# morisUtokyo/mTR

Measured on AMD Instinct MI355X. Metric: reads/sec, 2 kb Nanopore synthetic, higher is better.
Workload: dtype int32

## Files before the change

### mtr_amd/__init__.py

```python
from __future__ import annotations

import ctypes as C
import os
from typing import List, NamedTuple, Sequence

import numpy as np

HERE = os.path.dirname(os.path.abspath(__file__))
LIB_PATH = os.environ.get("MTR_LIB", os.path.join(HERE, "libmtr_hip.so"))
MAX_PERIOD = 500
MAX_READ_LENGTH = 833333
TEXT_ASCII, TEXT_CODES = 0, 1
FASTA_TILE_BYTES = 4096
FASTA_END = {0: "eof", 1: "empty", 2: "bad", 3: "toolong"}
FASTQ_END = {**FASTA_END, 4: "format", 5: "more"}

STATUS = {0: "MTR_OK", 1: "MTR_ERR_NO_DEVICE", 2: "MTR_ERR_BAD_ARG", 3: "MTR_ERR_OOM", 4: "MTR_ERR_HIP",
          5: "MTR_ERR_OVERFLOW", 6: "MTR_ERR_DP_TOO_LARGE"}
COUNTER_NAMES = ["dp_calls", "dp_cells", "dp_rows", "revise_dp_calls", "revise_dp_cells", "kmer_tables", "kmer_lookups",
                 "ranges_candidate", "ranges_executed", "records", "di_passes", "di_positions", "traceback_steps",
                 "undefined_guards", "global_tables", "reserved",
                 "cyc_total", "cyc_dp_fwd", "cyc_dp_tb", "cyc_tab_build", "cyc_seeds", "cyc_walk", "cyc_polish", "cyc_revise_vote",
                 "cyc_slot_copy", "cyc_dp_fwd_rev", "cyc_dp_tb_rev", "cyc_k1_codes", "cyc_k1_passes", "cyc_k1_extract",
                 "cyc_k1_dedup", "cyc_k1_total",
                 "memo_hits", "memo_cells", "tables_skipped", "cyc_tb_refill", "tb_refills", "walk_steps", "walk_slow_steps", "cyc_walk_slow",
                 "walk_calls", "walk_closed", "cyc_walk_fast", "prof43", "prof44", "prof45", "prof46", "prof47",
                 "qpass_bytes_dp2", "qpass_cells_dp2", "qpass_bytes_rev", "qpass_cells_rev", "revisions_shared", "reads_sent_back", "ranges_searched", "prof55"]
EXPORTS = ["mtr_create", "mtr_destroy", "mtr_last_error", "mtr_abi_version", "mtr_process_batch", "mtr_free_results",
           "mtr_upload_batch", "mtr_run_resident", "mtr_fetch_results", "mtr_get_kernel_times", "mtr_get_counters",
           "mtr_test_ranges", "mtr_test_ranges_parts", "mtr_test_wrap_dp", "mtr_test_wrap_dp_pass", "mtr_test_polish", "mtr_test_revise", "mtr_test_last_mode", "mtr_set_trace", "mtr_get_trace",
           "mtr_run_resident_async", "mtr_wait", "mtr_alignments",
           "mtr_file_state_create", "mtr_file_state_destroy", "mtr_upload_batch_in_file", "mtr_file_state_skip",
           "mtr_get_bases_after_read", "mtr_upload_batch_packed", "mtr_fetch_results_packed", "mtr_export_packed_device",
           "mtr_unpack_records", "mtr_pack_records", "mtr_get_first_failed_read", "mtr_upload_batch_device",
           "mtr_report_device", "mtr_test_chain", "mtr_report_alignments_device", "mtr_report_text_device", "mtr_test_report_lines",
           "mtr_parse_fasta_device", "mtr_upload_fasta_device", "mtr_fasta_index",
           "mtr_parse_fastq_device", "mtr_upload_fastq_device", "mtr_upload_fastq_device_in_file",
           "mtr_upload_batch_device_in_file", "mtr_upload_fasta_device_in_file", "mtr_file_state_skip_device", "mtr_test_file_tail",
           "mtr_parse_fasta_device_window", "mtr_upload_fasta_device_window", "mtr_parse_fastq_device_window", "mtr_upload_fastq_device_window",
           "mtr_report_motifs_device", "mtr_test_unit_motifs", "mtr_search_motifs_device",
           "mtr_search_motif_loci_device", "mtr_motif_loci_copy_device", "mtr_search_flanks_device", "mtr_genotype_loci_device",
           "mtr_call_alleles_device", "mtr_genotype_partial_device", "mtr_genotype_catalog_device", "mtr_genotype_catalog_copy_device",
           "mtr_call_alleles_rows_device", "mtr_test_catalog_stats", "mtr_genotype_partial_catalog_device", "mtr_genotype_partial_catalog_copy_device",
           "mtr_test_partial_catalog_stats", "mtr_catalog_create", "mtr_catalog_destroy", "mtr_catalog_info_get", "mtr_genotype_catalog_prepared_device",
           "mtr_genotype_partial_catalog_prepared_device", "mtr_test_catalog_dump", "mtr_test_catalog_build_stats",
           "mtr_extract_windows_device", "mtr_allele_consensus_device", "mtr_window_structure_device",
           "mtr_window_edits_device", "mtr_window_edits_copy_device", "mtr_test_window_edits_rounds"]
WE_FIELDS = 6
WS_MAX_SEGMENTS, WS_MAX_WINDOW = 4, 16384
CONS_MAX_WINDOW, CONS_MAX_BAND, CONS_INS_SLOTS, CONS_MAX_EXTRA = 16384, 256, 4, 64
ALLELE_COPIES, ALLELE_BASES = 0, 1
ALIGN_WIDTH = 50


class MtrError(RuntimeError):
    pass


class FileState:

    def __init__(self):
        self.lib = load_library()
        h = C.c_void_p()
        st = self.lib.mtr_file_state_create(C.byref(h))
        if st != 0:
            raise MtrError(f"mtr_file_state_create: {STATUS.get(st, st)}")
        self.h = h

    def skip(self, reads):
        bases, offs, lens = _flatten(reads)
        st = self.lib.mtr_file_state_skip(self.h, bases.ctypes.data, offs.ctypes.data, lens.ctypes.data, len(reads))
        if st != 0:
            raise MtrError(f"mtr_file_state_skip: {STATUS.get(st, st)}")

    def skip_device(self, engine: "Engine", text, offsets, lens, codes: bool = False):
        import torch

        offs, ln = device_input_args(text, offsets, lens, engine.device)
        stream = torch.cuda.current_stream(text.device).cuda_stream
        engine._check(self.lib.mtr_file_state_skip_device(engine.h, self.h, C.c_void_p(text.data_ptr()), text.numel(), offs.ctypes.data, ln.ctypes.data,
                                                          len(ln), TEXT_CODES if codes else TEXT_ASCII, C.c_void_p(stream)), "mtr_file_state_skip_device")

    def close(self):
# ... 401 lines not shown
    if not os.path.exists(path):
        raise MtrError(f"{path} is missing: build it with `python -m mtr_amd.build` (hipcc, gfx950); there is no CPU fallback")
    lib = C.CDLL(path)
    P = C.POINTER
    lib.mtr_create.argtypes = [C.c_int, C.c_int, C.c_float, P(C.c_void_p)]
    lib.mtr_create.restype = C.c_int
    lib.mtr_destroy.argtypes = [C.c_void_p]
    lib.mtr_destroy.restype = None
    lib.mtr_last_error.argtypes = [C.c_void_p]
    lib.mtr_last_error.restype = C.c_char_p
    lib.mtr_abi_version.restype = C.c_int
    lib.mtr_process_batch.argtypes = [C.c_void_p, C.c_void_p, C.c_void_p, C.c_void_p, C.c_int32, P(P(CRecord)), P(P(C.c_int32)), P(C.c_int64)]
    lib.mtr_process_batch.restype = C.c_int
    lib.mtr_free_results.argtypes = [C.c_void_p, C.c_void_p]
    lib.mtr_free_results.restype = None
    lib.mtr_upload_batch.argtypes = [C.c_void_p, C.c_void_p, C.c_void_p, C.c_void_p, C.c_int32]
    lib.mtr_upload_batch.restype = C.c_int
    lib.mtr_run_resident.argtypes = [C.c_void_p]
    lib.mtr_run_resident.restype = C.c_int
    lib.mtr_file_state_create.argtypes = [P(C.c_void_p)]
    lib.mtr_file_state_create.restype = C.c_int
    lib.mtr_file_state_destroy.argtypes = [C.c_void_p]
    lib.mtr_file_state_destroy.restype = None
    lib.mtr_upload_batch_in_file.argtypes = [C.c_void_p, C.c_void_p, C.c_void_p, C.c_void_p, C.c_void_p, C.c_int32]
    lib.mtr_upload_batch_in_file.restype = C.c_int
    lib.mtr_file_state_skip.argtypes = [C.c_void_p, C.c_void_p, C.c_void_p, C.c_void_p, C.c_int32]
    lib.mtr_file_state_skip.restype = C.c_int
    lib.mtr_run_resident_async.argtypes = [C.c_void_p]
    lib.mtr_run_resident_async.restype = C.c_int
    lib.mtr_wait.argtypes = [C.c_void_p]
    lib.mtr_wait.restype = C.c_int
    lib.mtr_test_last_mode.argtypes = [C.c_void_p]
    lib.mtr_test_last_mode.restype = C.c_int32
    lib.mtr_fetch_results.argtypes = [C.c_void_p, P(P(CRecord)), P(P(C.c_int32)), P(C.c_int64)]
    lib.mtr_fetch_results.restype = C.c_int
    lib.mtr_get_kernel_times.argtypes = [C.c_void_p, P(CKernelTime), C.c_int32]
    lib.mtr_get_kernel_times.restype = C.c_int
    lib.mtr_alignments.argtypes = [C.c_void_p, C.c_int32, P(C.c_int32), C.c_void_p, P(P(C.c_uint8)), P(P(C.c_int64)), P(P(C.c_int32))]
    lib.mtr_alignments.restype = C.c_int
    lib.mtr_get_counters.argtypes = [C.c_void_p, P(C.c_int64), C.c_int32]
    lib.mtr_get_counters.restype = C.c_int
    lib.mtr_test_ranges.argtypes = [C.c_void_p, P(P(C.c_int32)), P(P(C.c_int32)), P(P(C.c_int32)), P(P(C.c_int32)), P(P(C.c_uint64)), P(C.c_int64)]
    lib.mtr_test_ranges.restype = C.c_int
    lib.mtr_test_ranges_parts.argtypes = lib.mtr_test_ranges.argtypes
    lib.mtr_test_ranges_parts.restype = C.c_int
    lib.mtr_test_wrap_dp.argtypes = [C.c_void_p, C.c_int32] + [C.c_void_p] * 9
    lib.mtr_test_wrap_dp.restype = C.c_int
    lib.mtr_test_wrap_dp_pass.argtypes = [C.c_void_p, C.c_int32, C.c_int32] + [C.c_void_p] * 10
    lib.mtr_test_wrap_dp_pass.restype = C.c_int
    lib.mtr_test_polish.argtypes = [C.c_void_p, C.c_int32] + [C.c_void_p] * 9
    lib.mtr_test_polish.restype = C.c_int
    lib.mtr_test_revise.argtypes = [C.c_void_p, C.c_int32, C.c_int32] + [C.c_void_p] * 6 + [C.c_int32] + [C.c_void_p] * 3
    lib.mtr_test_revise.restype = C.c_int
    lib.mtr_upload_batch_packed.argtypes = [C.c_void_p, C.c_void_p, C.c_int64, C.c_void_p, C.c_void_p, C.c_int32]
    lib.mtr_upload_batch_packed.restype = C.c_int
    lib.mtr_upload_batch_device.argtypes = [C.c_void_p, C.c_void_p, C.c_int64, C.c_void_p, C.c_void_p, C.c_int32, C.c_int32, C.c_void_p]
    lib.mtr_upload_batch_device.restype = C.c_int
    lib.mtr_fetch_results_packed.argtypes = [C.c_void_p, C.c_int32, P(C.c_void_p), P(C.c_int64), P(C.c_void_p), P(C.c_int64)]
    lib.mtr_fetch_results_packed.restype = C.c_int
    lib.mtr_export_packed_device.argtypes = [C.c_void_p, C.c_void_p, C.c_int64, C.c_void_p, P(C.c_int64), P(C.c_int64)]
    lib.mtr_export_packed_device.restype = C.c_int
    lib.mtr_report_device.argtypes = [C.c_void_p, P(CReportDst), C.c_void_p, P(C.c_int64), P(C.c_int64)]
    lib.mtr_report_device.restype = C.c_int
    lib.mtr_report_alignments_device.argtypes = [C.c_void_p, P(CReportAlignDst), P(C.c_int64), P(C.c_int64)]
    lib.mtr_report_alignments_device.restype = C.c_int
    lib.mtr_report_text_device.argtypes = [C.c_void_p, C.c_void_p, C.c_void_p, C.c_int32, P(CReportTextDst), P(C.c_int64)]
    lib.mtr_report_text_device.restype = C.c_int
    lib.mtr_report_motifs_device.argtypes = [C.c_void_p, P(CReportMotifDst), P(C.c_int64), P(C.c_int64), P(C.c_int64)]
    lib.mtr_report_motifs_device.restype = C.c_int
    lib.mtr_test_unit_motifs.argtypes = ([C.c_void_p, C.c_int32] + [C.c_void_p] * 5 + [C.c_int64, P(P(C.c_uint8))] + [P(P(C.c_int32))] * 3 +
                                         [P(C.c_int64), P(P(C.c_int64)), P(P(C.c_uint8))] + [P(P(C.c_int32))] * 3 + [P(P(C.c_int64))] * 2)
    lib.mtr_test_unit_motifs.restype = C.c_int
    lib.mtr_search_motifs_device.argtypes = [C.c_void_p, C.c_void_p, C.c_void_p] + [C.c_int32] * 5 + [P(CMotifHitsDst), P(C.c_int64)]
    lib.mtr_search_motifs_device.restype = C.c_int
    lib.mtr_search_motif_loci_device.argtypes = [C.c_void_p, C.c_void_p, C.c_void_p] + [C.c_int32] * 7 + [P(C.c_int64), P(C.c_int64)]
    lib.mtr_search_motif_loci_device.restype = C.c_int
    lib.mtr_motif_loci_copy_device.argtypes = [C.c_void_p, P(CMotifLociDst)]
    lib.mtr_motif_loci_copy_device.restype = C.c_int
    lib.mtr_search_flanks_device.argtypes = [C.c_void_p, C.c_void_p, C.c_void_p, C.c_int32, C.c_int32, P(CFlankHitsDst), P(C.c_int64)]
    lib.mtr_search_flanks_device.restype = C.c_int
    lib.mtr_genotype_loci_device.argtypes = [C.c_void_p, C.c_void_p, C.c_void_p] + [C.c_int32] * 5 + [P(CGenotypesDst), P(C.c_int64)]
    lib.mtr_genotype_loci_device.restype = C.c_int
    lib.mtr_genotype_catalog_device.argtypes = [C.c_void_p, C.c_void_p, C.c_void_p] + [C.c_int32] * 6 + [P(C.c_int64), P(C.c_int64)]
    lib.mtr_genotype_catalog_device.restype = C.c_int
    lib.mtr_genotype_catalog_copy_device.argtypes = [C.c_void_p, P(CCatalogDst)]
    lib.mtr_genotype_catalog_copy_device.restype = C.c_int
    lib.mtr_genotype_partial_device.argtypes = [C.c_void_p, C.c_void_p, C.c_void_p] + [C.c_int32] * 6 + [P(CPartialDst), P(C.c_int64)]
    lib.mtr_genotype_partial_device.restype = C.c_int
    lib.mtr_genotype_partial_catalog_device.argtypes = [C.c_void_p, C.c_void_p, C.c_void_p] + [C.c_int32] * 7 + [P(C.c_int64), P(C.c_int64)]
    lib.mtr_genotype_partial_catalog_device.restype = C.c_int
    lib.mtr_genotype_partial_catalog_copy_device.argtypes = [C.c_void_p, P(CPartialCatalogDst)]
    lib.mtr_genotype_partial_catalog_copy_device.restype = C.c_int
    if hasattr(lib, "mtr_catalog_create"):
        lib.mtr_catalog_create.argtypes = [C.c_void_p, C.c_void_p, C.c_void_p, C.c_int32, C.c_int32, C.c_int32, P(C.c_void_p)]
        lib.mtr_catalog_create.restype = C.c_int
        lib.mtr_catalog_destroy.argtypes = [C.c_void_p]
        lib.mtr_catalog_destroy.restype = None
        lib.mtr_catalog_info_get.argtypes = [C.c_void_p, P(CCatalogInfo)]
        lib.mtr_catalog_info_get.restype = C.c_int
        lib.mtr_genotype_catalog_prepared_device.argtypes = [C.c_void_p, C.c_void_p] + [C.c_int32] * 3 + [P(C.c_int64), P(C.c_int64)]
        lib.mtr_genotype_catalog_prepared_device.restype = C.c_int
        lib.mtr_genotype_partial_catalog_prepared_device.argtypes = [C.c_void_p, C.c_void_p] + [C.c_int32] * 4 + [P(C.c_int64), P(C.c_int64)]
        lib.mtr_genotype_partial_catalog_prepared_device.restype = C.c_int
        lib.mtr_test_catalog_dump.argtypes = [C.c_void_p, C.c_void_p, P(CCatalogDump)]
        lib.mtr_test_catalog_dump.restype = C.c_int
        lib.mtr_test_catalog_build_stats.argtypes = [C.c_void_p, P(C.c_double)]
# ... 1025 lines not shown
    @staticmethod
    def _dp_task_arrays(tasks, pad_units: bool):
        rd = np.array([t[0] for t in tasks], np.int32)
        qs = np.array([t[1] for t in tasks], np.int32)
        qe = np.array([t[2] for t in tasks], np.int32)
        uo = np.zeros(len(tasks) + 1, np.int32)
        uo[1:] = np.cumsum([len(t[3]) for t in tasks])
        units = np.ascontiguousarray(np.concatenate([np.asarray(t[3], np.uint8) for t in tasks] + ([np.zeros(1, np.uint8)] if pad_units else [])))
        g = np.array([t[4] for t in tasks], np.int32)
        m = np.array([t[5] for t in tasks], np.int32)
        d = np.array([t[6] for t in tasks], np.int32)
        return rd, qs, qe, units, uo, g, m, d

    def test_wrap_dp(self, tasks):
        n = len(tasks)
        arrays = self._dp_task_arrays(tasks, pad_units=False)
        out = np.zeros((n, 8), np.int32)
        self._check(self.lib.mtr_test_wrap_dp(self.h, n, *(a.ctypes.data for a in arrays), out.ctypes.data), "mtr_test_wrap_dp")
        return out

    def test_polish(self, tasks):
        n = len(tasks)
        rd, rs, re, kk = (np.array([t[i] for t in tasks], np.int32) for i in range(4))
        uo = np.zeros(n + 1, np.int32)
        uo[1:] = np.cumsum([len(t[4]) for t in tasks])
        units = np.ascontiguousarray(np.concatenate([np.asarray(t[4], np.uint8) for t in tasks]))
        scores = np.ascontiguousarray(np.concatenate([np.asarray(t[5], np.int32) for t in tasks]))
        out_units, out_len = np.zeros((n, 500), np.uint8), np.zeros(n, np.int32)
        self._check(self.lib.mtr_test_polish(self.h, n, rd.ctypes.data, rs.ctypes.data, re.ctypes.data, kk.ctypes.data, units.ctypes.data,
                                             scores.ctypes.data, uo.ctypes.data, out_units.ctypes.data, out_len.ctypes.data), "mtr_test_polish")
        return [out_units[i, :out_len[i]].copy() for i in range(n)]

    REVISE_MODES = {"WAVE": 0, "SLOTS": 1}

    def test_revise(self, mode: str, groups, waves: int = 0):
        tasks = [t for g in groups for t in g]
        n = len(tasks)
        go = np.zeros(len(groups) + 1, np.int32)
        go[1:] = np.cumsum([len(g) for g in groups])
        rd = np.array([t[0] for t in tasks] + [0], np.int32)
        rr = np.ascontiguousarray(np.array([list(t[1]) for t in tasks] + [[0] * 13], np.int32).reshape(-1, 13))
        uo = np.zeros(n + 1, np.int32)
        uo[1:] = np.cumsum([len(t[2]) for t in tasks])
        units = np.ascontiguousarray(np.concatenate([np.asarray(t[2], np.uint8) for t in tasks] + [np.zeros(1, np.uint8)]))
        scores = np.ascontiguousarray(np.concatenate([np.asarray(t[3], np.int32) for t in tasks] + [np.zeros(1, np.int32)]))
        if any(len(t[2]) != len(t[3]) for t in tasks):
            raise ValueError("a task's node frequencies are one per unit base")
        out_rr, out_units, cells = np.zeros((max(n, 1), 13), np.int32), np.zeros((max(n, 1), 500), np.uint8), C.c_int64(0)
        self._check(self.lib.mtr_test_revise(self.h, self.REVISE_MODES[mode], len(groups), go.ctypes.data, rd.ctypes.data, rr.ctypes.data, units.ctypes.data,
                                             scores.ctypes.data, uo.ctypes.data, int(waves), out_rr.ctypes.data, out_units.ctypes.data, C.byref(cells)),
                    "mtr_test_revise")
        return [(tuple(int(v) for v in out_rr[i]), out_units[i, :max(0, min(int(out_rr[i, 3]), 500))].copy()) for i in range(n)], int(cells.value)

    DP_PASSES = {"WAVE2P": 0, "Q4": 1, "QUAD2P": 2, "FOUR1P": 3, "OCT1P": 4, "OCT2P": 5}

    def test_wrap_dp_pass(self, dp_pass: str, groups):
        tasks = [t for g in groups for t in g]
        n = len(tasks)
        go = np.zeros(len(groups) + 1, np.int32)
        go[1:] = np.cumsum([len(g) for g in groups])
        arrays = self._dp_task_arrays(tasks, pad_units=True)
        out = np.zeros((max(n, 1), 2, 8), np.int32)
        self._check(self.lib.mtr_test_wrap_dp_pass(self.h, self.DP_PASSES[dp_pass], len(groups), go.ctypes.data, *(a.ctypes.data for a in arrays), out.ctypes.data),
                    "mtr_test_wrap_dp_pass")
        return out[:n]

    def set_trace(self, max_events: int):
        self._check(self.lib.mtr_set_trace(self.h, max_events), "mtr_set_trace")

    def get_trace(self) -> np.ndarray:
        ev = C.POINTER(C.c_int32)()
        n = C.c_int64()
        self._check(self.lib.mtr_get_trace(self.h, C.byref(ev), C.byref(n)), "mtr_get_trace")
        arr = np.ctypeslib.as_array(ev, shape=(max(n.value, 1), 16))[: n.value].copy()
        _libc.free(C.cast(ev, C.c_void_p))
        return arr


def _c_float_text(x) -> str:
    x = float(x)
    if x != x:
        return "-nan" if np.signbit(x) else "nan"
    if x in (float("inf"), float("-inf")):
        return "inf" if x > 0 else "-inf"
    return "%f" % x


def format_report(ids, lens, report: Report, alignments: "ReportAlignments | None" = None) -> bytes:
    def host(t):
        return t.detach().cpu().numpy() if hasattr(t, "detach") else np.asarray(t)

    read, fields, ratio = host(report.read), host(report.fields).reshape(-1, 14), host(report.ratio).astype(np.float32)
    unit_off, units = host(report.unit_off), host(report.units).tobytes()
    if alignments is not None:
        col_off, text = host(alignments.col_off), np.ascontiguousarray(host(alignments.text), np.uint8)
        text = text.reshape(3, text.size // 3)
        rows = [text[0].tobytes(), text[1].tobytes(), text[2].tobytes()]
        if len(col_off) != len(read) + 1:
            raise MtrError(f"alignments of {len(col_off) - 1} repeats for a report of {len(read)}")
    out = []
    bid = [i.encode() if isinstance(i, str) else bytes(i) for i in ids]
    for k in range(len(read)):
        r = int(read[k])
        f = [int(v) for v in fields[k]]
        cols = [str(int(lens[r])), str(f[0] + 1), str(f[1] + 1), str(f[2]), str(f[3]), str(f[4]), str(f[5]), _c_float_text(ratio[k]),
                str(f[6]), str(f[7]), str(f[8])]
# ... 451 lines not shown
```

### mtr_amd/csrc/dp_test.hip.inc

```
#pragma once
#include "dp_wrap.hip.inc"

struct DpPassArgs {
    DpTestArgs t;
    int32_t pass, n_groups;
    const int32_t *group_off;
    long long packed_words;
};

DEVINL void dpt_clear(DpRes &o) { o.stop_i = 0; o.end_i = 0; o.mat = o.mis = o.ins = o.del = o.scanned = 0; o.end_j = 0; }
DEVINL void dpt_store(const DpPassArgs &a, int task, int p, int qs, int U, const DpRes &o)
{
    if (lane_id() == 0) {
        int32_t *r = a.t.out8 + ((size_t)task * 2 + (size_t)p) * 8;
        r[0] = qs + o.stop_i + 1; r[1] = qs + o.end_i; r[2] = o.end_i - o.stop_i; r[3] = U > 0 ? o.scanned / U : 0;
        r[4] = o.mat; r[5] = o.mis; r[6] = o.ins; r[7] = o.del;
    }
}
template <int FMT>
DEVINL void dpt_traceback(const DpPassArgs &a, const uint32_t *pk, int qs, int U, const uint8_t *cells, int psel, int rstride, const int (&best)[3],
                          DpRes &o, unsigned long long *wc)
{
    dpt_clear(o);
    const int bv = uni(best[0]), bi = uni(best[1]), bj = uni(best[2]);
// ... 144 lines not shown
        }
        wave_sync_mem();
        loop_join();
    }
    wc_flush(s_cnt, a.t.counters);
}

__global__ __launch_bounds__(64, MTR_WAVES_PER_SIMD) void mtr_k_dp_test_rev(DpPassArgs a)
{
    __shared__ unsigned long long s_cnt[CNT_N];
    if (lane_id() < CNT_N) s_cnt[lane_id()] = 0ull;
    uint8_t *cells = a.t.scratch + (size_t)blockIdx.x * a.t.scratch_per_wave;
    for (;;) {
        const int grp = next_work_item(a.t.work_counter);
        if (grp >= a.n_groups) break;
        const int t0 = uni(a.group_off[grp]), n = uni(a.group_off[grp + 1]) - t0;
        DpOct q; q.n = n;
        int maxrows = 0, maxU = 0;
#pragma unroll 1
        for (int g = 0; g < RQ_SLOTS; g++) { q.pk[g] = a.t.b.packed; q.wlim[g] = 1; q.base[g] = 0; q.rows[g] = 0; q.U[g] = 0; q.unit[g] = cells; q.G[g] = 1; q.MM[g] = 1; q.D[g] = 1; }
#pragma unroll 1
        for (int k = 0; k < n; k++) {
            const int tg = t0 + k;
            const int rd = uni(a.t.read_idx[tg]), uo = uni(a.t.unit_off[tg]);
            q.pk[k] = a.t.b.packed + uni64(a.t.b.woff[rd]); q.wlim[k] = a.packed_words - uni64(a.t.b.woff[rd]);
            q.base[k] = uni(a.t.qs[tg]); q.rows[k] = uni(a.t.qe[tg]) - q.base[k] + 1;
            q.U[k] = uni(a.t.unit_off[tg + 1]) - uo; q.unit[k] = a.t.units + uo;
            q.G[k] = uni(a.t.gain[tg]); q.MM[k] = uni(a.t.mism[tg]); q.D[k] = uni(a.t.indel[tg]);
            maxrows = q.rows[k] > maxrows ? q.rows[k] : maxrows; maxU = q.U[k] > maxU ? q.U[k] : maxU;
        }
        const int Cq = DPQ_COLS(maxU);
        int best[RQ_SLOTS][3];
        for (int g = 0; g < RQ_SLOTS; g++) { best[g][0] = 0; best[g][1] = 0; best[g][2] = 0; }
        if (a.pass == MTR_TEST_PASS_FOUR1P) st_fwd1p_four(Cq, q, cells, maxrows, best); else st_fwd1p_any(Cq, q, cells, maxrows, best);
        wave_sync_mem();
#pragma unroll 1
        for (int k = 0; k < n; k++) {
            int bk[3] = { best[0][0], best[0][1], best[0][2] };
#pragma unroll
            for (int h = 1; h < RQ_SLOTS; h++) if (k == h) { bk[0] = best[h][0]; bk[1] = best[h][1]; bk[2] = best[h][2]; }
            const int tg = t0 + k;
            const int rd = uni(a.t.read_idx[tg]), qs = uni(a.t.qs[tg]), U = uni(a.t.unit_off[tg + 1]) - uni(a.t.unit_off[tg]);
            DpRes o;
            dpt_traceback<3>(a, a.t.b.packed + uni64(a.t.b.woff[rd]), qs, U, cells + (size_t)k * DPQP_DP_BYTES(Cq, maxrows), 0, DPQ_ROW_BYTES(Cq), bk, o, s_cnt);
            dpt_store(a, tg, 0, qs, U, o);
            loop_join();
        }
        wave_sync_mem();
        loop_join();
    }
    wc_flush(s_cnt, a.t.counters);
}

struct PolishTestArgs {
    K2Args a;
    int32_t n_tasks;
    const int32_t *read_idx, *rep_start, *rep_end, *k;
    const uint8_t *units; const int32_t *scores, *unit_off;
    uint8_t *out_units; int32_t *out_len;
};
__global__ __launch_bounds__(64, MTR_LAT_WAVES_PER_SIMD) void mtr_k_polish_test(PolishTestArgs p)
{
    __shared__ __attribute__((aligned(16))) int s_arena[MTR_ARENA_INTS];
    __shared__ unsigned long long s_cnt[CNT_N];
    int *s_keys = s_arena, *s_seeds = s_arena + K2_TAB_CAP, *s_stage = s_seeds + MTRC_MAX_SEEDS + 4;
    const int lane = lane_id();
    if (lane < CNT_N) s_cnt[lane] = 0ull;
    K2Ctx c;
    c.a = &p.a; c.wc = s_cnt;
    c.sc = p.a.scratch + (size_t)blockIdx.x * p.a.scratch_per_wave;
    c.y = k2_layout(p.a.Lmax, p.a.cells_cap);
    c.lds_keys = (lds_int *)s_keys; c.seeds = (lds_int *)s_seeds; c.stage = (lds_int *)s_stage;
    c.ties = (int *)(c.sc + c.y.ties); c.fresh = c.ties + MTRC_MAX_TIEBREAKS;
    c.memo_n = 0; c.memo_qs = c.memo_qe = -1; c.memo_U = 0; c.rmemo_n = 0;
    for (;;) {
        const int t = next_work_item(p.a.work_counter);
        if (t >= p.n_tasks) break;
        st_member_ctx(c, p.a, uni(p.read_idx[t]));
        const int uo = uni(p.unit_off[t]), U = uni(p.unit_off[t + 1]) - uo;
        RR r; rr_clear(r);
        r.rep_start = uni(p.rep_start[t]); r.rep_end = uni(p.rep_end[t]); r.kmer = uni(p.k[t]); r.period = U;
        uint8_t *ub = slot_unit(c, 1);
        slot_load_candidate(ub, slot_score(c, 1), p.units + uo, p.scores + uo, U);
        wave_sync_mem();
        polish(c, r, 1);
#pragma unroll 1
        for (int q = lane; q < r.period; q += 64) p.out_units[(size_t)t * MTRC_MAX_PERIOD + q] = ub[q];
        if (lane == 0) p.out_len[t] = r.period;
        wave_sync_mem();
        loop_join();
    }
    wc_flush(s_cnt, p.a.counters);
}

struct ReviseTestArgs {
    K2Args a;
    int32_t n_groups;
    const int32_t *group_off, *read_idx, *rr;
    const uint8_t *units; const int32_t *scores, *unit_off;
    int32_t *out_rr; uint8_t *out_units;
};
__global__ __launch_bounds__(64, MTR_WAVES_PER_SIMD) void mtr_k_revise_test(ReviseTestArgs p)
{
    __shared__ __attribute__((aligned(16))) int s_arena[MTR_ARENA_INTS];
    __shared__ unsigned long long s_cnt[CNT_N];
    int *s_keys = s_arena, *s_seeds = s_arena + K2_TAB_CAP, *s_stage = s_seeds + MTRC_MAX_SEEDS + 4;
// ... 37 lines not shown
```

### mtr_amd/csrc/dp_wrap.hip.inc

```
#pragma once
#include "device_util.hip.inc"
#include "dp_quad.hip.inc"

struct DpRes { int stop_i, end_i, mat, mis, ins, del, scanned, end_j; };

template <int NCH>
DEVINL void dp_forward(const uint32_t *pk, int base, int rows, const uint8_t *unit, int U, int G, int MM, int D,
                       uint8_t *codes, int &best_v, int &best_i, int &best_j)
{
    const int lane = lane_id();
    int u[NCH], P[NCH], bv[NCH], bi[NCH];
#pragma unroll
    for (int c = 0; c < NCH; c++) {
        int j0 = 64 * c + lane;
        u[c] = (j0 < U) ? (int)unit[j0] : -1;
        P[c] = 0; bv[c] = 0; bi[c] = 0;
    }
    {
        int landed = 0;
#pragma unroll
        for (int c = 0; c < NCH; c++) landed += lane_val(u[c], 0);
        asm volatile("" :: "s"(landed));
    }
    const int last_c = (U - 1) >> 6, last_l = (U - 1) & 63;
// ... 621 lines not shown
    const uint32_t e0 = __builtin_amdgcn_alignbyte(d1, d0, sh), e1 = __builtin_amdgcn_alignbyte(d2, d1, sh);
    const uint32_t e2 = d2 >> (8 * sh);
    unsigned long long v = ((unsigned long long)e1 << 32) | (unsigned long long)e0;
    if (c & 1) v = (v >> 4) | ((unsigned long long)(e2 & 0xFu) << 60);
    return v;
}

struct TbOps { uint8_t *ops; int cap; int n; int overflow; };
template <int MODE, int FMT>
DEVINL void dp_traceback(const uint32_t *pk, int base, int U, const uint8_t *codes, int psel, int rstride, int bi, int bj,
                         int *cons, int *miss, lds_int *lv, DpRes &res, unsigned long long *counters, TbOps *out = nullptr)
{
    const int lane = lane_id();
    int i = bi, j = bj;
    int mat = 0, mis = 0, ins = 0, del = 0;
    long guard = ((long)bi + 1) * ((long)U + 1);
    const float invU = 1.0f / (float)U;
    const int KU = __mul24((int)(256.0f * invU) + 1, U);
    auto mod_U = [&](int x) {
        const int y = x + KU;
        int r = y - __mul24((int)((float)y * invU), U);
        r = r < 0 ? r + U : r;
        return r >= U ? r - U : r;
    };
    for (;;) {
        const int i_top = i;
        const int row = i_top - lane;
        const unsigned long long t_refill = clk();
        unsigned long long q64 = 0ull;
        int xr = 0;
        if (row >= 1) {
            const int NS = FMT == 1 ? 4 * psel : FMT == 3 ? 4 * ((row - 1) & 1) : 0;
            const uint8_t *rp = codes + (size_t)(FMT == 3 ? (row - 1) >> 1 : row - 1) * (size_t)rstride;
            const int c = mod_U(j - 1 - lane - TB_SLACK);
            q64 = FMT == 2 ? tb_cells16_nibbles(rp, c) : tb_cells16_bytes(rp + c, NS);
            if (c + 16 > U) {
                const int n1 = U - c;
                const unsigned long long wrap = FMT == 2 ? tb_cells16_nibbles(rp, 0) : tb_cells16_bytes(rp, NS);
                q64 = (q64 & ((1ull << (4 * n1)) - 1ull)) | (wrap << (4 * n1));
                if (U < 16) {
                    q64 &= (1ull << (4 * U)) - 1ull;
                    for (int sh = 4 * U; sh < 64; sh *= 2) q64 |= q64 << sh;
                }
            }
            if (MODE == 1) xr = base_at(pk, base + row);
        }
        {
            int landed = lane_val((int)((unsigned)q64 ^ (unsigned)(q64 >> 32)) ^ xr, 0);
            asm volatile("" :: "s"(landed));
        }
        wc_time(counters, CYC_TB_REFILL, t_refill);
        wc_add(counters, CNT_TB_REFILLS, 1);
        const int r_max = i_top - 1 < 63 ? i_top - 1 : 63;
        int r = 0, t4 = 4 * TB_SLACK, jj = j;
        int wm = 0, wx = 0, wd = 0, wn = 0;
        for (;;) {
            const int cl = (int)((unsigned)(q64 >> t4) & 15u);
            const unsigned long long mM = __ballot(DPC_IS_M(cl)), mX = __ballot(DPC_IS_X(cl));
            const unsigned long long dg = (mM | mX) >> r;
            const unsigned long long seg0 = dg & ~(dg + 1ull);
            const int run = __builtin_popcountll(seg0);
            if (MODE == 0) {
                const unsigned long long seg = seg0 << r;
                wm += __builtin_popcountll(mM & seg); wx += __builtin_popcountll(mX & seg);
                r += run;
                if (r > r_max) { if (i_top - r <= 0) goto tb_last; break; }
                const int code = lane_val(cl, r);
                if (DPC_IS_Z(code)) goto tb_last;
                const int isdel = (code & 4) ? 0 : 1;
                wd += isdel; wn += 1 - isdel;
                t4 += 4 - 8 * isdel; r += 1 - isdel;
                if (r > r_max) { if (i_top - r <= 0) goto tb_last; break; }
                if ((unsigned)t4 > 60u) break;
                continue;
            }
            if (run > 0) {
                const unsigned long long seg = seg0 << r;
                wm += __builtin_popcountll(mM & seg); wx += __builtin_popcountll(mX & seg);
                if (MODE == 2) {
                    if (out->n + run > out->cap) { out->overflow = 1; goto tb_last; }
                    if (lane >= r && lane < r + run) out->ops[out->n + (lane - r)] = DPC_IS_M(cl) ? (uint8_t)1 : (uint8_t)2;
                    out->n += run;
                }
                if (MODE == 1) {
                    if (lane >= r && lane < r + run) {
                        int jl = jj - (lane - r);
                        if (U >= 64) jl = jl < 1 ? jl + U : jl; else jl = mod_U(jl - 1) + 1;
                        tb_vote(lv, cons, 0, jl * 5 + xr);
                    }
                    jj -= run;
                    if (U >= 64) jj = jj < 1 ? jj + U : jj; else { while (jj < 1) jj += U; }
                }
                r += run;
                if (r > r_max) { if (i_top - r <= 0) goto tb_last; break; }
            }
            const int code = lane_val(cl, r);
            if (DPC_IS_Z(code)) goto tb_last;
            if ((code & 4) == 0) {
                if (MODE == 1) { if (lane == 0) tb_vote(lv, cons, 0, jj * 5 + 4); jj -= 1; if (jj < 1) jj = U; }
                if (MODE == 2) { if (out->n + 1 > out->cap) { out->overflow = 1; goto tb_last; } if (lane == 0) out->ops[out->n] = 3; out->n += 1; }
                wd++; t4 -= 4;
                if (t4 < 0) break;
            } else {
                if (MODE == 1 && lane == r) tb_vote(lv, miss, (U + 1) * 5, jj * 4 + xr);
                if (MODE == 2) { if (out->n + 1 > out->cap) { out->overflow = 1; goto tb_last; } if (lane == 0) out->ops[out->n] = 4; out->n += 1; }
                wn++; t4 += 4; r++;
                if (r > r_max) { if (i_top - r <= 0) goto tb_last; break; }
                if (t4 > 60) break;
            }
            if (MODE != 0) loop_join();
        }
        mat += wm; mis += wx; del += wd; ins += wn;
        i = i_top - r;
        if (MODE == 1) j = jj;
        else j = mod_U(j - 1 - (wm + wx + wd)) + 1;
        guard -= (long)(wm + wx + wd + wn) + 1;
        if (guard < 0) break;
        loop_join();
        continue;
    tb_last:
        mat += wm; mis += wx; del += wd; ins += wn;
        i = i_top - r;
        if (MODE == 1) j = jj;
        guard -= (long)(wm + wx + wd + wn) + 1;
        break;
    }
    res.stop_i = guard < 0 ? -1 : i; res.end_i = bi; res.mat = mat; res.mis = mis; res.ins = ins; res.del = del; res.scanned = mat + mis + del;
}

DEVINL bool dp_wrap2_fits(int rows, int U, int lim16)
{
    return U <= 128 || (U <= 256 && rows <= DP2P_MAX_ROWS && rows <= lim16);
}
DEVINL bool dp_wrap2(const uint32_t *pk, int base, int rows, const uint8_t *unit, int U,
                     int G0, int MM0, int D0, int G1, int MM1, int D1,
                     uint8_t *codes, size_t codes_cap, DpRes (&res)[2], unsigned long long *counters, int lim16)
{
    for (int d = 0; d < 2; d++) { res[d].stop_i = 0; res[d].end_i = 0; res[d].mat = res[d].mis = res[d].ins = res[d].del = res[d].scanned = 0; }
    base = uni(base); rows = uni(rows); U = uni(U);
    if (U <= 0 || rows <= 0) return true;
    if (!dp_size_ok(U, rows)) return false;
    const size_t cells = (size_t)rows * (size_t)U;
    const bool packed = rows <= DP2P_MAX_ROWS && rows <= lim16;
    const bool two_col = packed && U > 64 && U <= 128 && (size_t)rows * (size_t)((U + 1) & ~1) <= codes_cap;
    const int c64 = DPQ_COLS64(U);
    const bool wide = packed && U > 128 && U <= 256 && DPQ_DP_BYTES_G(64, c64, rows) <= codes_cap;
    const int rstride = two_col ? (U + 1) & ~1 : wide ? DPQ_ROW_BYTES_G(64, c64) : U;
    if ((packed ? (size_t)rows * (size_t)rstride : 2 * cells) > codes_cap) return false;
    int best[2][3];
    const unsigned long long t_f = clk();
    if (!packed && U > 128) return false;
    if (packed) {
        if (U <= 64) dp_forward2p<1>(pk, base, rows, unit, U, G0, MM0, D0, G1, MM1, D1, codes, best);
        else if (two_col) dp_forward2p_2c(pk, base, rows, unit, U, G0, MM0, D0, G1, MM1, D1, codes, rstride, best);
        else if (U <= 128) dp_forward2p<2>(pk, base, rows, unit, U, G0, MM0, D0, G1, MM1, D1, codes, best);
        else if (wide) {
            DpQuad q; q.n = 1;
            q.pk[0] = pk; q.wlim[0] = (long long)((base + rows) >> 4) + 2; q.base[0] = base; q.rows[0] = rows; q.U[0] = U; q.unit[0] = unit;
            int b4[4][2][3];
            if (c64 == 3) dp_forward2p_g16<3, 64, 1>(q, G0, MM0, D0, G1, MM1, D1, codes, rows, b4);
            else dp_forward2p_g16<4, 64, 1>(q, G0, MM0, D0, G1, MM1, D1, codes, rows, b4);
            for (int d = 0; d < 2; d++) for (int k = 0; k < 3; k++) best[d][k] = b4[0][d][k];
        }
        else dp_forward2p<4>(pk, base, rows, unit, U, G0, MM0, D0, G1, MM1, D1, codes, best);
    } else {
        if (U <= 64) dp_forward2<1>(pk, base, rows, unit, U, G0, MM0, D0, G1, MM1, D1, codes, codes + cells, best);
        else dp_forward2<2>(pk, base, rows, unit, U, G0, MM0, D0, G1, MM1, D1, codes, codes + cells, best);
    }
    wave_sync_mem();
    wc_time(counters, CYC_DP_FWD, t_f);
    if (U <= 16) wc_time_aux(counters, CNT_SPARE47, t_f);
    const unsigned long long t_b = clk();
    bool ok = true;
    for (int d = 0; d < 2; d++) {
        const int bv = uni(best[d][0]), bi = uni(best[d][1]), bj = uni(best[d][2]);
        if (bv > 0) {
// ... 87 lines not shown
```

### mtr_amd/csrc/revise_task.h

```cpp
#pragma once
#include <cstdint>
#include <string>

#define RVT_MIN_PERIOD 6
#define RVT_MAX_PERIOD 499
#define RVT_MIN_COVERAGE 5
#define RVT_MAX_COVERAGE 20
#define RVT_MIN_K 2
#define RVT_MAX_K 15
#define RVT_MAX_TASKS 4096

inline std::string rvt_refusal(int32_t rd, int32_t n_reads, const int32_t *lens, const int32_t *rr, int64_t unit_len, long long wrap_dp_size)
{
    if (rd < 0 || rd >= n_reads) return "read outside the batch";
    const long long L = lens[rd];
    const long long rs = rr[0], re = rr[1], repeat_len = rr[2], period = rr[3], k = rr[9];
    if (period < RVT_MIN_PERIOD || period > RVT_MAX_PERIOD) return "period outside 6..499";
    if (unit_len != period) return "the unit's length is not the period";
    if (rs < 0 || re < rs || re > L) return "window outside 0 <= rep_start <= rep_end <= L";
    if (rr[5] < 0 || rr[6] < 0 || rr[7] < 0 || rr[8] < 0 || (long long)rr[5] + rr[6] + rr[7] + rr[8] <= 0 || repeat_len <= 0) return "non-positive counts";
    const long long coverage = repeat_len / period;
    if (coverage < RVT_MIN_COVERAGE || coverage > RVT_MAX_COVERAGE) return "coverage outside 5..20";
    if (k < RVT_MIN_K || k > RVT_MAX_K) return "k outside 2..15";
    if ((2 * period + 1) * (re - rs + 1) + 2 * period >= wrap_dp_size) return "period x rows beyond WrapDPsize";
    return std::string();
}
```

Measured before the change: 307,200.

## Batch traceback votes per refill window instead of per step in vote mode

In vote mode (MODE 1), traceback now runs the same fast diagonal-run loop as MODE 0. It records each lane's row code offset and the positions of deletions, then casts all consensus and miss votes in parallel across lanes once per 64-row refill window. This removes the per-step serialized voting, column bookkeeping and loop joins in the slow path. It also adds a test kernel that compares global and LDS vote tables against the ops traceback. The risk is that the reconstructed vote columns differ from the old step-by-step ones, and the deletion count per window is capped at 64.

```diff
diff --git a/mtr_amd/__init__.py b/mtr_amd/__init__.py
--- a/mtr_amd/__init__.py
+++ b/mtr_amd/__init__.py
@@ -28,7 +28,7 @@
                  "qpass_bytes_dp2", "qpass_cells_dp2", "qpass_bytes_rev", "qpass_cells_rev", "revisions_shared", "reads_sent_back", "ranges_searched", "prof55"]
 EXPORTS = ["mtr_create", "mtr_destroy", "mtr_last_error", "mtr_abi_version", "mtr_process_batch", "mtr_free_results",
            "mtr_upload_batch", "mtr_run_resident", "mtr_fetch_results", "mtr_get_kernel_times", "mtr_get_counters",
-           "mtr_test_ranges", "mtr_test_ranges_parts", "mtr_test_wrap_dp", "mtr_test_wrap_dp_pass", "mtr_test_polish", "mtr_test_revise", "mtr_test_last_mode", "mtr_set_trace", "mtr_get_trace",
+           "mtr_test_ranges", "mtr_test_ranges_parts", "mtr_test_wrap_dp", "mtr_test_wrap_dp_pass", "mtr_test_polish", "mtr_test_revise", "mtr_test_vote_traceback", "mtr_test_last_mode", "mtr_set_trace", "mtr_get_trace",
            "mtr_run_resident_async", "mtr_wait", "mtr_alignments",
            "mtr_file_state_create", "mtr_file_state_destroy", "mtr_upload_batch_in_file", "mtr_file_state_skip",
            "mtr_get_bases_after_read", "mtr_upload_batch_packed", "mtr_fetch_results_packed", "mtr_export_packed_device",
@@ -536,6 +536,9 @@
     lib.mtr_test_polish.restype = C.c_int
     lib.mtr_test_revise.argtypes = [C.c_void_p, C.c_int32, C.c_int32] + [C.c_void_p] * 6 + [C.c_int32] + [C.c_void_p] * 3
     lib.mtr_test_revise.restype = C.c_int
+    if hasattr(lib, "mtr_test_vote_traceback"):
+        lib.mtr_test_vote_traceback.argtypes = [C.c_void_p, C.c_int32] + [C.c_void_p] * 13
+        lib.mtr_test_vote_traceback.restype = C.c_int
     lib.mtr_upload_batch_packed.argtypes = [C.c_void_p, C.c_void_p, C.c_int64, C.c_void_p, C.c_void_p, C.c_int32]
     lib.mtr_upload_batch_packed.restype = C.c_int
     lib.mtr_upload_batch_device.argtypes = [C.c_void_p, C.c_void_p, C.c_int64, C.c_void_p, C.c_void_p, C.c_int32, C.c_int32, C.c_void_p]
@@ -1667,6 +1670,28 @@
                     "mtr_test_revise")
         return [(tuple(int(v) for v in out_rr[i]), out_units[i, :max(0, min(int(out_rr[i, 3]), 500))].copy()) for i in range(n)], int(cells.value)
 
+    VTB_OUT_INTS, VTB_STRIDE = 32, 9 * 501
+
+    def test_vote_traceback(self, tasks):
+        n = len(tasks)
+        arrays = self._dp_task_arrays(tasks, pad_units=True)
+        fmt = np.array([t[7] for t in tasks] + [0], np.int32)
+        oo = np.zeros(n + 1, np.int64)
+        oo[1:] = np.cumsum([2 * (t[2] - t[1] + 1) + 2 * len(t[3]) + 64 for t in tasks])
+        out = np.zeros((max(n, 1), self.VTB_OUT_INTS), np.int32)
+        votes = np.zeros((max(n, 1), 2, self.VTB_STRIDE), np.int32)
+        ops = np.zeros(max(int(oo[-1]), 1), np.uint8)
+        self._check(self.lib.mtr_test_vote_traceback(self.h, n, *(a.ctypes.data for a in arrays), fmt.ctypes.data, oo.ctypes.data, out.ctypes.data,
+                                                     votes.ctypes.data, ops.ctypes.data), "mtr_test_vote_traceback")
+        res = []
+        for i, t in enumerate(tasks):
+            u1 = len(t[3]) + 1
+            tabs = [(votes[i, v, :5 * u1].reshape(u1, 5).copy(), votes[i, v, 5 * u1:9 * u1].reshape(u1, 4).copy()) for v in range(2)]
+            res.append({"best": tuple(int(v) for v in out[i, 0:3]), "ops": ops[oo[i]:oo[i] + out[i, 3]].copy(),
+                        "cons": tabs[0][0], "miss": tabs[0][1], "cons_lds": tabs[1][0], "miss_lds": tabs[1][1],
+                        "res": tuple(int(v) for v in out[i, 8:15]), "res_lds": tuple(int(v) for v in out[i, 16:23]), "res_ops": tuple(int(v) for v in out[i, 24:31])})
+        return res
+
     DP_PASSES = {"WAVE2P": 0, "Q4": 1, "QUAD2P": 2, "FOUR1P": 3, "OCT1P": 4, "OCT2P": 5}
 
     def test_wrap_dp_pass(self, dp_pass: str, groups):
diff --git a/mtr_amd/csrc/dp_test.hip.inc b/mtr_amd/csrc/dp_test.hip.inc
--- a/mtr_amd/csrc/dp_test.hip.inc
+++ b/mtr_amd/csrc/dp_test.hip.inc
@@ -220,6 +220,95 @@
     wc_flush(s_cnt, a.t.counters);
 }
 
+#define VTB_STRIDE (9 * (MTRC_MAX_PERIOD + 1))
+#define VTB_OUT_INTS 32
+struct VoteTbArgs {
+    DpTestArgs t;
+    const long long *ops_off, *fmt;
+    int32_t *votes; uint8_t *ops;
+    long long packed_words;
+};
+DEVINL void vtb_store(int32_t *r, const DpRes &o)
+{
+    r[0] = o.stop_i; r[1] = o.end_i; r[2] = o.mat; r[3] = o.mis; r[4] = o.ins; r[5] = o.del; r[6] = o.scanned;
+}
+template <int FMT>
+DEVINL void vtb_tracebacks(const uint32_t *pk, int base, int U, const uint8_t *cells, int rstride, int bi, int bj, int *cons, int *miss, lds_int *lv,
+                           DpRes (&o)[3], TbOps &out, unsigned long long *wc)
+{
+    dp_traceback<1, FMT>(pk, base, U, cells, 0, rstride, bi, bj, cons, miss, nullptr, o[0], wc);
+    dp_traceback<1, FMT>(pk, base, U, cells, 0, rstride, bi, bj, nullptr, nullptr, lv, o[1], wc);
+    dp_traceback<2, FMT>(pk, base, U, cells, 0, rstride, bi, bj, nullptr, nullptr, nullptr, o[2], wc, &out);
+}
+__global__ __launch_bounds__(64, MTR_WAVES_PER_SIMD) void mtr_k_vote_tb_test(VoteTbArgs a)
+{
+    __shared__ unsigned long long s_cnt[CNT_N];
+    __shared__ int s_votes[16 + VTB_STRIDE];
+    const int lane = lane_id();
+    if (lane < CNT_N) s_cnt[lane] = 0ull;
+    uint8_t *cells = a.t.scratch + (size_t)blockIdx.x * a.t.scratch_per_wave;
+    lds_int *lv = (lds_int *)s_votes + 16;
+    for (;;) {
+        const int t = next_work_item(a.t.work_counter);
+        if (t >= a.t.n_tasks) break;
+        const int rd = uni(a.t.read_idx[t]), uo = uni(a.t.unit_off[t]), U = uni(a.t.unit_off[t + 1]) - uo;
+        const uint32_t *pk = a.t.b.packed + uni64(a.t.b.woff[rd]);
+        const int base = uni(a.t.qs[t]) - 1, rows = uni(a.t.qe[t]) - base;
+        const uint8_t *unit = a.t.units + uo;
+        const int G = uni(a.t.gain[t]), MM = uni(a.t.mism[t]), D = uni(a.t.indel[t]);
+        const int fmt = (int)uni64(a.fmt[t]);
+        int bv = 0, bi = 0, bj = 0, rstride = U;
+        if (fmt == 0) {
+            if (U <= 64) dp_forward<1>(pk, base, rows, unit, U, G, MM, D, cells, bv, bi, bj);
+            else if (U <= 128) dp_forward<2>(pk, base, rows, unit, U, G, MM, D, cells, bv, bi, bj);
+            else if (U <= 256) dp_forward<4>(pk, base, rows, unit, U, G, MM, D, cells, bv, bi, bj);
+            else dp_forward<8>(pk, base, rows, unit, U, G, MM, D, cells, bv, bi, bj);
+        } else if (U <= ST_QUMAX) {
+            DpOct q; q.n = 1;
+#pragma unroll 1
+            for (int g = 0; g < RQ_SLOTS; g++) { q.pk[g] = a.t.b.packed; q.wlim[g] = 1; q.base[g] = 0; q.rows[g] = 0; q.U[g] = 0; q.unit[g] = cells; q.G[g] = 1; q.MM[g] = 1; q.D[g] = 1; }
+            q.pk[0] = pk; q.wlim[0] = a.packed_words - uni64(a.t.b.woff[rd]); q.base[0] = base; q.rows[0] = rows; q.U[0] = U; q.unit[0] = unit; q.G[0] = G; q.MM[0] = MM; q.D[0] = D;
+            const int Cq = DPQ_COLS(U);
+            int best[RQ_SLOTS][3];
+            for (int g = 0; g < RQ_SLOTS; g++) { best[g][0] = 0; best[g][1] = 0; best[g][2] = 0; }
+            st_fwd1p_four(Cq, q, cells, rows, best);
+            bv = best[0][0]; bi = best[0][1]; bj = best[0][2]; rstride = DPQ_ROW_BYTES(Cq);
+        } else {
+            const int c64 = DPQ_COLS64(U);
+            DpQuad q; q.n = 1;
+            q.pk[0] = pk; q.wlim[0] = a.packed_words - uni64(a.t.b.woff[rd]); q.base[0] = base; q.rows[0] = rows; q.U[0] = U; q.unit[0] = unit; q.G[0] = G; q.MM[0] = MM; q.D[0] = D;
+            int b4[4][3];
+            if (c64 == 3) dp_forward1p_g16<3, 64, 1, true>(q, cells, rows, b4); else dp_forward1p_g16<4, 64, 1, true>(q, cells, rows, b4);
+            bv = b4[0][0]; bi = b4[0][1]; bj = b4[0][2]; rstride = DPQ_ROW_BYTES_G(64, c64);
+        }
+        for (int k = lane; k < (U + 1) * 9; k += 64) lv[k] = 0;
+        wave_sync_mem();
+        bv = uni(bv); bi = uni(bi); bj = uni(bj);
+        DpRes o[3];
+        for (int k = 0; k < 3; k++) dpt_clear(o[k]);
+        const long long oo = uni64(a.ops_off[t]);
+        TbOps out = { a.ops + oo, (int)(uni64(a.ops_off[t + 1]) - oo), 0, 0 };
+        int *cons = a.votes + (size_t)(2 * t) * VTB_STRIDE, *miss = cons + (U + 1) * 5;
+        if (bv > 0) {
+            if (fmt == 0) vtb_tracebacks<0>(pk, base, U, cells, rstride, bi, bj, cons, miss, lv, o, out, s_cnt);
+            else vtb_tracebacks<3>(pk, base, U, cells, rstride, bi, bj, cons, miss, lv, o, out, s_cnt);
+            if (o[0].stop_i < 0 || o[1].stop_i < 0 || o[2].stop_i < 0) set_status(a.t.status, DEV_ERR_DP_TOO_LARGE);
+            if (out.overflow) set_status(a.t.status, DEV_ERR_RECORD_OVERFLOW);
+        }
+        wave_sync_mem();
+        int32_t *lo = a.votes + (size_t)(2 * t + 1) * VTB_STRIDE;
+        for (int k = lane; k < (U + 1) * 9; k += 64) lo[k] = lv[k];
+        if (lane == 0) {
+            int32_t *r = a.t.out8 + (size_t)t * VTB_OUT_INTS;
+            r[0] = bv; r[1] = bi; r[2] = bj; r[3] = out.n;
+            vtb_store(r + 8, o[0]); vtb_store(r + 16, o[1]); vtb_store(r + 24, o[2]);
+        }
+        wave_sync_mem();
+        loop_join();
+    }
+    wc_flush(s_cnt, a.t.counters);
+}
+
 struct PolishTestArgs {
     K2Args a;
     int32_t n_tasks;
diff --git a/mtr_amd/csrc/dp_wrap.hip.inc b/mtr_amd/csrc/dp_wrap.hip.inc
--- a/mtr_amd/csrc/dp_wrap.hip.inc
+++ b/mtr_amd/csrc/dp_wrap.hip.inc
@@ -697,15 +697,29 @@
         wc_time(counters, CYC_TB_REFILL, t_refill);
         wc_add(counters, CNT_TB_REFILLS, 1);
         const int r_max = i_top - 1 < 63 ? i_top - 1 : 63;
-        int r = 0, t4 = 4 * TB_SLACK, jj = j;
+        int r = 0, t4 = 4 * TB_SLACK;
         int wm = 0, wx = 0, wd = 0, wn = 0;
+        int rec = 0, park = 0;
+        auto cast_votes = [&]() {
+            if (lane < r) {
+                const int cr = (int)((unsigned)(q64 >> rec) & 15u);
+                const int col = mod_U(j - 1 - lane - TB_SLACK + (rec >> 2)) + 1;
+                const bool dgl = DPC_IS_M(cr) || DPC_IS_X(cr);
+                tb_vote(lv, dgl ? cons : miss, dgl ? 0 : (U + 1) * 5, dgl ? col * 5 + xr : col * 4 + xr);
+            }
+            if (lane < wd) {
+                const int col = mod_U(j - 1 - TB_SLACK + (park >> 2)) + 1;
+                tb_vote(lv, cons, 0, col * 5 + 4);
+            }
+        };
         for (;;) {
             const int cl = (int)((unsigned)(q64 >> t4) & 15u);
             const unsigned long long mM = __ballot(DPC_IS_M(cl)), mX = __ballot(DPC_IS_X(cl));
             const unsigned long long dg = (mM | mX) >> r;
             const unsigned long long seg0 = dg & ~(dg + 1ull);
             const int run = __builtin_popcountll(seg0);
-            if (MODE == 0) {
+            if (MODE != 2) {
+                if (MODE == 1) rec = lane >= r ? t4 : rec;
                 const unsigned long long seg = seg0 << r;
                 wm += __builtin_popcountll(mM & seg); wx += __builtin_popcountll(mX & seg);
                 r += run;
@@ -713,60 +727,48 @@
                 const int code = lane_val(cl, r);
                 if (DPC_IS_Z(code)) goto tb_last;
                 const int isdel = (code & 4) ? 0 : 1;
+                if (MODE == 1) park = write_lane(park, t4 - 4 * r, wd);
                 wd += isdel; wn += 1 - isdel;
                 t4 += 4 - 8 * isdel; r += 1 - isdel;
                 if (r > r_max) { if (i_top - r <= 0) goto tb_last; break; }
-                if ((unsigned)t4 > 60u) break;
+                if ((unsigned)(MODE == 1 ? t4 | (wd & 64) : t4) > 60u) break;
                 continue;
             }
             if (run > 0) {
                 const unsigned long long seg = seg0 << r;
                 wm += __builtin_popcountll(mM & seg); wx += __builtin_popcountll(mX & seg);
-                if (MODE == 2) {
-                    if (out->n + run > out->cap) { out->overflow = 1; goto tb_last; }
-                    if (lane >= r && lane < r + run) out->ops[out->n + (lane - r)] = DPC_IS_M(cl) ? (uint8_t)1 : (uint8_t)2;
-                    out->n += run;
-                }
-                if (MODE == 1) {
-                    if (lane >= r && lane < r + run) {
-                        int jl = jj - (lane - r);
-                        if (U >= 64) jl = jl < 1 ? jl + U : jl; else jl = mod_U(jl - 1) + 1;
-                        tb_vote(lv, cons, 0, jl * 5 + xr);
-                    }
-                    jj -= run;
-                    if (U >= 64) jj = jj < 1 ? jj + U : jj; else { while (jj < 1) jj += U; }
-                }
+                if (out->n + run > out->cap) { out->overflow = 1; goto tb_last; }
+                if (lane >= r && lane < r + run) out->ops[out->n + (lane - r)] = DPC_IS_M(cl) ? (uint8_t)1 : (uint8_t)2;
+                out->n += run;
                 r += run;
                 if (r > r_max) { if (i_top - r <= 0) goto tb_last; break; }
             }
             const int code = lane_val(cl, r);
             if (DPC_IS_Z(code)) goto tb_last;
             if ((code & 4) == 0) {
-                if (MODE == 1) { if (lane == 0) tb_vote(lv, cons, 0, jj * 5 + 4); jj -= 1; if (jj < 1) jj = U; }
-                if (MODE == 2) { if (out->n + 1 > out->cap) { out->overflow = 1; goto tb_last; } if (lane == 0) out->ops[out->n] = 3; out->n += 1; }
+                if (out->n + 1 > out->cap) { out->overflow = 1; goto tb_last; } if (lane == 0) out->ops[out->n] = 3; out->n += 1;
                 wd++; t4 -= 4;
                 if (t4 < 0) break;
             } else {
-                if (MODE == 1 && lane == r) tb_vote(lv, miss, (U + 1) * 5, jj * 4 + xr);
-                if (MODE == 2) { if (out->n + 1 > out->cap) { out->overflow = 1; goto tb_last; } if (lane == 0) out->ops[out->n] = 4; out->n += 1; }
+                if (out->n + 1 > out->cap) { out->overflow = 1; goto tb_last; } if (lane == 0) out->ops[out->n] = 4; out->n += 1;
                 wn++; t4 += 4; r++;
                 if (r > r_max) { if (i_top - r <= 0) goto tb_last; break; }
                 if (t4 > 60) break;
             }
-            if (MODE != 0) loop_join();
+            loop_join();
         }
         mat += wm; mis += wx; del += wd; ins += wn;
+        if (MODE == 1) cast_votes();
         i = i_top - r;
-        if (MODE == 1) j = jj;
-        else j = mod_U(j - 1 - (wm + wx + wd)) + 1;
+        j = mod_U(j - 1 - (wm + wx + wd)) + 1;
         guard -= (long)(wm + wx + wd + wn) + 1;
         if (guard < 0) break;
         loop_join();
         continue;
     tb_last:
         mat += wm; mis += wx; del += wd; ins += wn;
+        if (MODE == 1) cast_votes();
         i = i_top - r;
-        if (MODE == 1) j = jj;
         guard -= (long)(wm + wx + wd + wn) + 1;
         break;
     }
diff --git a/mtr_amd/csrc/revise_task.h b/mtr_amd/csrc/revise_task.h
--- a/mtr_amd/csrc/revise_task.h
+++ b/mtr_amd/csrc/revise_task.h
@@ -9,6 +9,15 @@
 #define RVT_MIN_K 2
 #define RVT_MAX_K 15
 #define RVT_MAX_TASKS 4096
+
+inline std::string rvt_dp_refusal(int32_t rd, int32_t n_reads, const int32_t *lens, long long rs, long long re, int64_t unit_len, long long wrap_dp_size)
+{
+    if (rd < 0 || rd >= n_reads) return "read outside the batch";
+    if (unit_len < RVT_MIN_PERIOD || unit_len > RVT_MAX_PERIOD) return "period outside 6..499";
+    if (rs < 0 || re < rs || re >= lens[rd]) return "window outside 0 <= start <= end < L";
+    if ((unit_len + 1) * (re - rs + 1) + unit_len >= wrap_dp_size) return "period x rows beyond WrapDPsize";
+    return std::string();
+}
 
 inline std::string rvt_refusal(int32_t rd, int32_t n_reads, const int32_t *lens, const int32_t *rr, int64_t unit_len, long long wrap_dp_size)
 {
```

Result: faster. 311,900, median of 6 (+1.5%).
